# rare-resilience-ai/Osteosarcoma_DiffusionModel

Measured on AMD Instinct MI355X. Metric: synthetic patients/sec (full T-step reverse sample), higher is better.
Workload: dtype f32; 1 GPU; reverse sampling of conditional patients, T=1000, D=2000 (50 mut + 1900 expr + 50 pathway), hidden [256,512,256], 3 scenario conditions (BASELINE config 3); patients_per_gpu=100000, T=1000, parallelism=patients sharded over 1 GPU(s), no collective, sampler=chain, chunk_rows=65536, streams=2, graph=True

## Files before the change

osteosarcoma_diffusionmodel_amd/csrc/chain.h:

```cpp
#pragma once
#include "gemm_glds.h"
#include "epilogues.h"
#include "xpose.h"
#include "launch.h"

namespace osd {

constexpr int CHAIN_MAX_LAYERS = 24;
enum : int { CK_INPUT = 0, CK_GN32 = 1, CK_GN64 = 2, CK_POST = 3 };
enum : unsigned { CHAIN_OK = 0, CHAIN_TIMEOUT = 1, CHAIN_ABORT = 2 };

struct ChainLayer {
  const float* A; int lda;
  int K, K0;
  int F;
  int in0, ld0, in1, ld1;
  int out, ldo;
  int kind;
  const float* bias; const float* gamma; const float* beta;
};

struct ChainArgs {
  ChainLayer L[CHAIN_MAX_LAYERS];
  int n_layers;
  float* ws; long long ws_stride;
  float* x; int D;
  int n, n_tiles;
  int t_first, n_steps;
  unsigned base_done;
  const float* cproj; int ldc;
  const float* temb; int ldt;
  const float* coef;
  const float* z; int ldzz; long long z_step_stride; int z_t_first;
  uint64_t seed; uint32_t row_offset;
  float* mut_mask; int mutation_dim;
  unsigned* progress;
  unsigned* status;
  unsigned* queue;
  unsigned* cu_arrivals;
  int stagger;
  unsigned long long spin_budget;
  unsigned long long* stamps;
};

typedef __attribute__((address_space(1))) unsigned gu32;

__device__ __forceinline__ unsigned ld_relaxed_agent(const unsigned* p) {
  return __hip_atomic_load(p, __ATOMIC_RELAXED, __HIP_MEMORY_SCOPE_AGENT);
}
__device__ __forceinline__ void st_relaxed_agent(unsigned* p, unsigned v) {
  __hip_atomic_store(p, v, __ATOMIC_RELAXED, __HIP_MEMORY_SCOPE_AGENT);
}

__device__ __forceinline__ bool chain_wait(const unsigned* word, unsigned want, unsigned* status, unsigned long long budget, int lane) {
  if ((unsigned)__builtin_amdgcn_readfirstlane((int)ld_relaxed_agent(word)) >= want) return true;
  const unsigned long long t0 = __builtin_amdgcn_s_memrealtime();
  for (;;) {
    __builtin_amdgcn_s_sleep(32);
    if ((unsigned)__builtin_amdgcn_readfirstlane((int)ld_relaxed_agent(word)) >= want) return true;
    if ((unsigned)__builtin_amdgcn_readfirstlane((int)ld_relaxed_agent(status)) != CHAIN_OK) return false;
    if (__builtin_amdgcn_s_memrealtime() - t0 > budget) {
      if (lane == 0) st_relaxed_agent(status, CHAIN_TIMEOUT);
      return false;
    }
  }
}

constexpr int CHAIN_PRM_FLOATS = 512;

template <int NPB>
struct XposeRowsOut {
  const WaveXpose<NPB>& xp; float* out; int ldo;
  __device__ __forceinline__ void put(int fb, int pb, int q, int l31, int h, float4 v) const { (void)fb; xp.put(pb, q, l31, h, v); }
  __device__ __forceinline__ void flush(int fb, int lane) const { xp.template store_rows<false>(out + 32 * fb, ldo, lane, 0, 0); }
};
template <int NPB>
struct XposeRowsIn {
  const WaveXpose<NPB>& xp; const float* src; int ld;
  __device__ __forceinline__ void load(int fb, int lane) const { xp.template load_rows<false>(src + 32 * fb, ld, lane, 0, 0); }
  __device__ __forceinline__ float4 get(int fb, int pb, int q, int l31, int h) const { (void)fb; return xp.get(pb, q, l31, h); }
};

template <int GW, int NFB, int NPB, int PS, class Out>
__device__ __forceinline__ void chain_gn_silu(f32x16 (&acc)[NFB][NPB], const float* __restrict__ prm, int fl, const Out& o, int lane,
                                              unsigned long long* ts = nullptr) {
  static_assert(GW >= 8 && NFB * 32 >= GW, "wave must own whole groups");
  constexpr int RPG = GW / 2;
  constexpr int NG = NFB * 16 / RPG;
  const int l31 = lane & 31, h = lane >> 5;
#pragma unroll
  for (int fb = 0; fb < NFB; ++fb)
#pragma unroll
    for (int q = 0; q < 4; ++q) {
      const float4 bv = *reinterpret_cast<const float4*>(prm + fl + 32 * fb + 8 * q + 4 * h);
#pragma unroll
      for (int pb = 0; pb < NPB; ++pb) {
        acc[fb][pb][4 * q] += bv.x; acc[fb][pb][4 * q + 1] += bv.y;
        acc[fb][pb][4 * q + 2] += bv.z; acc[fb][pb][4 * q + 3] += bv.w;
      }
    }
  if (ts) { asm volatile("s_waitcnt vmcnt(0) lgkmcnt(0)" ::: "memory"); ts[0] = __builtin_amdgcn_s_memtime(); }
  float mean[NPB][NG], rstd[NPB][NG];
#pragma unroll
  for (int pb = 0; pb < NPB; ++pb)
#pragma unroll
    for (int g = 0; g < NG; ++g) {
      float s = 0.f;
#pragma unroll
      for (int j = 0; j < RPG; ++j) { const int Li = g * RPG + j; s += acc[Li / 16][pb][Li % 16]; }
      s += swap_halves(s);
      const float m = s * (1.0f / GW);
      float qs = 0.f;
#pragma unroll
      for (int j = 0; j < RPG; ++j) { const int Li = g * RPG + j; const float d = acc[Li / 16][pb][Li % 16] - m; qs = fmaf(d, d, qs); }
      qs += swap_halves(qs);
      mean[pb][g] = m;
      rstd[pb][g] = 1.0f / sqrtf(qs * (1.0f / GW) + GN_EPS);
    }
  if (ts) { asm volatile("s_nop 0" ::: "memory"); ts[1] = __builtin_amdgcn_s_memtime(); ts[2] = ts[1]; }
#pragma unroll
  for (int fb = 0; fb < NFB; ++fb) {
#pragma unroll
    for (int q = 0; q < 4; ++q) {
      const int f = fl + 32 * fb + 8 * q + 4 * h;
      const float4 gv = *reinterpret_cast<const float4*>(prm + PS + f);
      const float4 bev = *reinterpret_cast<const float4*>(prm + 2 * PS + f);
      const int g = (fb * 16 + 4 * q) / RPG;
#pragma unroll
      for (int pb = 0; pb < NPB; ++pb) {
        const float m = mean[pb][g], r = rstd[pb][g];
        float4 y;
        y.x = silu_f(fmaf((acc[fb][pb][4 * q] - m) * r, gv.x, bev.x));
        y.y = silu_f(fmaf((acc[fb][pb][4 * q + 1] - m) * r, gv.y, bev.y));
        y.z = silu_f(fmaf((acc[fb][pb][4 * q + 2] - m) * r, gv.z, bev.z));
        y.w = silu_f(fmaf((acc[fb][pb][4 * q + 3] - m) * r, gv.w, bev.w));
        o.put(fb, pb, q, l31, h, y);
      }
    }
    o.flush(fb, lane);
  }
}

template <int NFB, int NPB, int PS, class In, class Out>
__device__ __forceinline__ void chain_input(f32x16 (&acc)[NFB][NPB], const float* __restrict__ prm, int fl, const In& in, const Out& o, int lane) {
  const int l31 = lane & 31, h = lane >> 5;
#pragma unroll
  for (int fb = 0; fb < NFB; ++fb) {
    in.load(fb, lane);
#pragma unroll
    for (int q = 0; q < 4; ++q) {
      const int f = fl + 32 * fb + 8 * q + 4 * h;
      const float4 bv = *reinterpret_cast<const float4*>(prm + f);
      const float4 tv = *reinterpret_cast<const float4*>(prm + PS + f);
#pragma unroll
      for (int pb = 0; pb < NPB; ++pb) {
        const float4 cv = in.get(fb, pb, q, l31, h);
        float4 v;
        v.x = ((acc[fb][pb][4 * q] + bv.x) + tv.x) + cv.x;
        v.y = ((acc[fb][pb][4 * q + 1] + bv.y) + tv.y) + cv.y;
        v.z = ((acc[fb][pb][4 * q + 2] + bv.z) + tv.z) + cv.z;
        v.w = ((acc[fb][pb][4 * q + 3] + bv.w) + tv.w) + cv.w;
        o.put(fb, pb, q, l31, h, v);
      }
    }
    o.flush(fb, lane);
  }
}

#ifndef OSD_EXP
#define OSD_EXP 0
#endif
template <int NFB, int NPB, bool PRE = false, bool GUARD = true>
__device__ __forceinline__ void chain_posterior(f32x16 (&acc)[NFB][NPB], const float* __restrict__ prm, int fl, float* __restrict__ x, int ldx,
                                                int prow, int pcol, float cA, float cB, float cC, int t, const float* __restrict__ zrow, int ldzz,
                                                uint64_t seed, uint32_t row_id0, int f_glob, float* __restrict__ mut_mask, int mutation_dim,
                                                const WaveXpose<NPB>& xp, int lane, float4 (*pre)[4 * NPB] = nullptr) {
  const int l31 = lane & 31, h = lane >> 5;
  if (prow <= 0) return;
  const bool do_mask = t == 0 && mut_mask != nullptr;
#pragma unroll
  for (int fb = 0; fb < NFB; ++fb) {
    const int cols = pcol - 32 * fb;
    if (GUARD && cols <= 0) break;
    if constexpr (PRE) {
      if (!(OSD_EXP & 2)) {
        xp.commit_rows(*pre, lane);
        if (fb + 1 < NFB && cols - 32 > 0) xp.template issue_rows<GUARD>(*pre, x + 32 * (fb + 1), ldx, lane, prow, cols - 32);
      }
    } else {
      xp.template load_rows<GUARD>(x + 32 * fb, ldx, lane, prow, cols);
    }
#pragma unroll
    for (int pb = 0; pb < NPB; ++pb) {
      const int p = 32 * pb + l31;
      const int pc = (!GUARD || p < prow) ? p : prow - 1;
#pragma unroll
      for (int q = 0; q < 4; ++q) {
        const int fo = 32 * fb + 8 * q + 4 * h;
        const float4 bv = *reinterpret_cast<const float4*>(prm + fl + fo);
        const float e[4] = {acc[fb][pb][4 * q] + bv.x, acc[fb][pb][4 * q + 1] + bv.y, acc[fb][pb][4 * q + 2] + bv.z, acc[fb][pb][4 * q + 3] + bv.w};
        const float4 xq = xp.get(pb, q, l31, h);
        const float xv[4] = {xq.x, xq.y, xq.z, xq.w};
        float4 zz = make_float4(0.f, 0.f, 0.f, 0.f);
        if (t > 0 && cC != 0.f) {
          if (zrow) {
            const int fc = (!GUARD || fo < pcol - 4) ? fo : pcol - 4;
            zz = ldg4(zrow + (size_t)pc * ldzz + fc);
          } else if (!(OSD_EXP & 1)) {
            zz = randn4(seed, row_id0 + (uint32_t)p, (uint32_t)((f_glob + fo) >> 2), (uint32_t)t, TAG_POSTERIOR);
          }
        }
        const float zv[4] = {zz.x, zz.y, zz.z, zz.w};
        float o[4];
#pragma unroll
        for (int r = 0; r < 4; ++r) o[r] = fmaf(cA, xv[r], fmaf(cB, e[r], cC * zv[r]));
        if (do_mask && p < prow && fo < pcol && f_glob + fo < mutation_dim) {
          float* mrow = mut_mask + (size_t)p * mutation_dim;
#pragma unroll
          for (int r = 0; r < 4; ++r)
            if (f_glob + fo + r < mutation_dim) stg1(mrow + f_glob + fo + r, (o[r] > 0.5f) ? 1.0f : 0.0f);
        }
        xp.put(pb, q, l31, h, make_float4(o[0], o[1], o[2], o[3]));
      }
    }
    if (!(OSD_EXP & 4)) xp.template store_rows<GUARD>(x + 32 * fb, ldx, lane, prow, cols);
  }
}

#ifndef CHAIN_EPI_PRIO
#define CHAIN_EPI_PRIO 0
#endif
#ifndef CHAIN_BP
#define CHAIN_BP 128
#endif
#if CHAIN_BP == 128
typedef Tile<128, 128, 64, 64> ChainTile;
constexpr int CHAIN_WPS = 2;
#else
typedef Tile<128, 64, 64, 32> ChainTile;
constexpr int CHAIN_WPS = 3;
#endif
#ifdef OSD_DIAG
constexpr int CHAIN_KCNT = 12;
constexpr int CHAIN_STAMP_FLOATS = 2 * 4 * CHAIN_KCNT;
#else
constexpr int CHAIN_KCNT = 10;
constexpr int CHAIN_STAMP_FLOATS = 80;
#endif
constexpr int CHAIN_PRM_OFF = 2 * (ChainTile::BF * BK + ChainTile::BP * BK) + 4 + CHAIN_STAMP_FLOATS;
constexpr int CHAIN_LDS_BYTES = (CHAIN_PRM_OFF + 2 * CHAIN_PRM_FLOATS) * 4;
static_assert(CHAIN_PRM_OFF % 4 == 0, "parameter blocks are read as float4");

template <bool STAMP>
__global__ __launch_bounds__(NTHREADS, CHAIN_WPS) void chain_kernel(const ChainArgs* __restrict__ gp) {
  const ChainArgs& a = *gp;
  typedef ChainTile T;
  typedef GldsTile<T> G;
  static_assert(T::BF == 128 && T::BP % 32 == 0, "staging below assumes a 128-row weight image");
  constexpr int NW = NTHREADS / 64;
  constexpr int NPW = 16 / NW;
  constexpr int NPWB = T::BP / 8 / NW;
  constexpr int PROWS = 8 * NW;
  constexpr unsigned PBYTES = 1024u * NW;
  extern __shared__ __attribute__((aligned(16))) float smem[];
  float* As0 = smem;
  float* As1 = smem + G::A_ELEMS;
  float* Bs0 = smem + 2 * G::A_ELEMS;
  float* Bs1 = smem + 2 * G::A_ELEMS + G::B_ELEMS;
  volatile int& s_flag = *reinterpret_cast<volatile int*>(smem + 2 * (G::A_ELEMS + G::B_ELEMS));

  const int tid = threadIdx.x;
  const int lane = tid & 63;
  const int wave = __builtin_amdgcn_readfirstlane(tid >> 6);
  const int wf = (wave / T::NWP) * T::WF;
  const int wp = (wave % T::NWP) * T::WP;

  float* const ws = a.ws + (long long)blockIdx.x * a.ws_stride;
  WaveXpose<T::NPB> xp;
  {
    const int xo = wave * (T::NPB * 1024);
    xp.buf = xo < G::A_ELEMS ? As1 + xo : Bs1 + (xo - G::A_ELEMS);
  }
  float* const prm_base = smem + CHAIN_PRM_OFF;
  int pcur = 0;

  if (a.cu_arrivals && a.stagger > 0) {
    if (wave == 0) {
      const unsigned hw = __builtin_amdgcn_s_getreg(0xF804);
      const unsigned xcc = __builtin_amdgcn_s_getreg(0xF814) & 7;
      const unsigned key = (xcc << 8) | ((hw >> 8) & 0xFF);
      unsigned r = 0;
      if (lane == 0) r = atomicAdd(a.cu_arrivals + key, 1u);
      s_flag = __builtin_amdgcn_readfirstlane((int)(r & 1u));
    }
    __syncthreads();
    const int late = __builtin_amdgcn_readfirstlane(s_flag);
    __syncthreads();
    if (late) {
      const unsigned long long t0 = __builtin_amdgcn_s_memtime();
      while (__builtin_amdgcn_s_memtime() - t0 < (unsigned long long)a.stagger) __builtin_amdgcn_s_sleep(16);
    }
  }

  unsigned long long c_dep = 0, c_pro = 0, c_k = 0, c_epi = 0, c_units = 0;
  unsigned long long* const kcnt = reinterpret_cast<unsigned long long*>(smem + 2 * (G::A_ELEMS + G::B_ELEMS) + 4);
  if constexpr (STAMP) {
    if (tid < 4 * CHAIN_KCNT) kcnt[tid] = 0;
    __syncthreads();
  }
  const unsigned long long c_start = STAMP ? __builtin_amdgcn_s_memtime() : 0;
  const long long n_units = (long long)a.n_tiles * a.n_steps;
  int c_iter = 0;
  (void)c_iter;
  for (;;) {
    const unsigned long long td0 = STAMP ? __builtin_amdgcn_s_memtime() : 0;
#ifdef CHAIN_STATIC_UNITS
    static_assert(true, "");
    const long long u = (long long)blockIdx.x + (long long)c_iter * gridDim.x;
    ++c_iter;
#else
    if (wave == 0) {
      unsigned nu = 0;
      if (lane == 0) nu = atomicAdd(a.queue, 1u);
      s_flag = __builtin_amdgcn_readfirstlane((int)nu);
    }
    __syncthreads();
    const long long u = (unsigned)__builtin_amdgcn_readfirstlane(s_flag);
    __syncthreads();
#endif
    if (u >= n_units) break;
    const int tile = (int)(u % a.n_tiles);
    const int si = (int)(u / a.n_tiles);
    const int t = a.t_first - si;
    const int p0 = tile * T::BP;
    const int P = (a.n - p0 < T::BP) ? a.n - p0 : T::BP;

    if (wave == 0) {
      bool ok = (unsigned)__builtin_amdgcn_readfirstlane((int)ld_relaxed_agent(a.status)) == CHAIN_OK;
      if (ok && si > 0) {
        ok = chain_wait(a.progress + tile, a.base_done + (unsigned)si, a.status, a.spin_budget, lane);
        if (ok) __builtin_amdgcn_fence(__ATOMIC_ACQUIRE, "agent");
      }
      s_flag = ok ? 1 : 0;
      asm volatile("s_waitcnt vmcnt(0) lgkmcnt(0)" ::: "memory");
    }
    __syncthreads();
    const int go = __builtin_amdgcn_readfirstlane(s_flag);
    if (!go) return;
    if constexpr (STAMP) { c_dep += __builtin_amdgcn_s_memtime() - td0; ++c_units; }

    auto first_stage = [&](const ChainLayer& Lr, int f0n, bool do_a, bool do_b, int pb) {
      struct { const float* A; int lda, F, in0, ld0, K0, K; } Ln{Lr.A, Lr.lda, Lr.F, Lr.in0, Lr.ld0, Lr.K0, Lr.K};
      if (do_a && wave < 2) {
        const int kind = Lr.kind;
        const float* src = Lr.bias;
        if (wave == 1) src = Lr.beta;
        else if (lane >= 32) src = kind == CK_INPUT ? a.temb + (size_t)t * a.ldt : (kind == CK_POST ? Lr.bias : Lr.gamma);
        if (wave == 0 || (kind != CK_INPUT && kind != CK_POST)) {
          int f = f0n + 4 * (lane & 31);
          f = f < Ln.F - 4 ? f : Ln.F - 4;
          glds16(src + f, __builtin_amdgcn_readfirstlane(lds_addr(prm_base + pb * CHAIN_PRM_FLOATS) + (unsigned)wave * 1024u));
        }
      }
      const float* const xrows = a.x + (size_t)p0 * a.D;
      int ln = lane;
      asm volatile("" : "+v"(ln));
      const int r0 = wave * 8 + (ln >> 3);
      const int k4 = 4 * ((ln & 7) ^ ((r0 >> 1) & 7));
      const unsigned la = __builtin_amdgcn_readfirstlane(lds_addr(As0) + (unsigned)wave * 1024u);
      const unsigned lb = __builtin_amdgcn_readfirstlane(lds_addr(Bs0) + (unsigned)wave * 1024u);
      if (do_a) {
#pragma unroll
        for (int j = 0; j < NPW; ++j) {
          int rg = f0n + r0 + PROWS * j;
          rg = rg < Ln.F ? rg : Ln.F - 1;
          glds16(Ln.A + (size_t)rg * Ln.lda + k4, __builtin_amdgcn_readfirstlane(la + (unsigned)j * PBYTES));
        }
      }
      if (do_b) {
        const bool from_x = Ln.in0 < 0;
        const float* bb = from_x ? xrows : ws + Ln.in0;
        const int rows = from_x ? P : T::BP;
        const int kend = Ln.K0 < Ln.K ? Ln.K0 : Ln.K;
        const int k = k4 < kend - 4 ? k4 : kend - 4;
#pragma unroll
        for (int j = 0; j < NPWB; ++j) {
          int rg = r0 + PROWS * j;
          rg = rg < rows ? rg : rows - 1;
          glds16(bb + (size_t)rg * Ln.ld0 + k, __builtin_amdgcn_readfirstlane(lb + (unsigned)j * PBYTES));
        }
      }
    };
    unsigned long long tt0 = STAMP ? __builtin_amdgcn_s_memtime() : 0;
    first_stage(a.L[0], 0, true, true, pcur);
    asm volatile("s_waitcnt vmcnt(0)" ::: "memory");
    __syncthreads();

    for (int l = 0; l < a.n_layers; ++l) {
      const ChainLayer& L = a.L[l];
      const gfloat_ptr LA = uniform_ptr(L.A);
      const int Llda = L.lda, LK0 = L.K0, Lld0 = L.ld0, Lld1 = L.ld1;
      const int F = L.F, K = L.K;
      const float* const B0g = (L.in0 < 0) ? a.x + (size_t)p0 * a.D : ws + L.in0;
      const float* const B1g = ws + L.in1;
      const gfloat_ptr B0 = uniform_ptr(B0g), B1 = uniform_ptr(B1g);
      const int rowsB = (L.in0 < 0) ? P : T::BP;
      const int nk = (K + BK - 1) / BK;
      const int nft = (F + T::BF - 1) / T::BF;
      for (int ft = 0; ft < nft; ++ft) {
        const int f0 = ft * T::BF;
        int ln = lane;
        asm volatile("" : "+v"(ln));
        const int l31 = ln & 31, h = ln >> 5;
        int st_row[NPW], st_k4[NPW];
#pragma unroll
        for (int j = 0; j < NPW; ++j) {
          st_row[j] = (j * NW + wave) * 8 + (ln >> 3);
          st_k4[j] = 4 * ((ln & 7) ^ ((st_row[j] >> 1) & 7));
        }
        int a_rd[T::NFB], a_sw[T::NFB], b_rd[T::NPB], b_sw[T::NPB];
#pragma unroll
        for (int fb = 0; fb < T::NFB; ++fb) { const int R = wf + 32 * fb + l31; a_rd[fb] = R * BK; a_sw[fb] = h ^ ((R >> 1) & 7); }
#pragma unroll
        for (int pb = 0; pb < T::NPB; ++pb) { const int R = wp + 32 * pb + l31; b_rd[pb] = R * BK; b_sw[pb] = h ^ ((R >> 1) & 7); }
        unsigned offA[NPW], offB[NPWB];
#pragma unroll
        for (int j = 0; j < NPW; ++j) {
          int rg = f0 + st_row[j];
          rg = rg < F ? rg : F - 1;
          offA[j] = (unsigned)(rg * Llda + st_k4[j]) * 4u;
        }
#pragma unroll
        for (int j = 0; j < NPWB; ++j) {
          int rb = st_row[j];
          rb = rb < rowsB ? rb : rowsB - 1;
          offB[j] = (unsigned)(rb * Lld0 + st_k4[j]) * 4u;
        }
        int b_panel = 0;
        auto b_offsets_for = [&](int k0) {
          const int want = k0 < LK0 ? 0 : 1;
          if (want != b_panel) {
            b_panel = want;
            const int ld = want ? Lld1 : Lld0;
#pragma unroll
            for (int j = 0; j < NPWB; ++j) {
              int rb = st_row[j];
              rb = rb < rowsB ? rb : rowsB - 1;
              offB[j] = (unsigned)(rb * ld + st_k4[j]) * 4u;
            }
          }
        };
        struct StageCtx { gfloat_ptr sa, sb; unsigned la, lb; int k0; bool tail; };
        auto stage_begin = [&](int k0, float* As, float* Bs) {
          b_offsets_for(k0);
          const bool first = k0 < LK0;
          const int kend = first ? (LK0 < K ? LK0 : K) : K - LK0;
          const int kl = first ? k0 : k0 - LK0;
          StageCtx c;
          c.sa = LA + __builtin_amdgcn_readfirstlane(k0);
          c.sb = (first ? B0 : B1) + __builtin_amdgcn_readfirstlane(kl);
          c.la = __builtin_amdgcn_readfirstlane(lds_addr(As) + (unsigned)wave * 1024u);
          c.lb = __builtin_amdgcn_readfirstlane(lds_addr(Bs) + (unsigned)wave * 1024u);
          c.k0 = k0;
          c.tail = kl + BK > kend;
          return c;
        };
        auto piece = [&](const StageCtx& c, int j) {
          if (j < NPW) glds16s(c.sa, offA[j], __builtin_amdgcn_readfirstlane(c.la + (unsigned)j * PBYTES));
          else glds16s(c.sb, offB[j - NPW], __builtin_amdgcn_readfirstlane(c.lb + (unsigned)(j - NPW) * PBYTES));
        };
        auto stage_tail = [&](const StageCtx& c) {
#pragma unroll
          for (int j = 0; j < NPW; ++j) piece(c, j);
          const bool first = c.k0 < LK0;
          const int kend = first ? (LK0 < K ? LK0 : K) : K - LK0;
          const int kl = first ? c.k0 : c.k0 - LK0;
          const float* bb = first ? B0g : B1g;
          const int ld = first ? Lld0 : Lld1;
#pragma unroll
          for (int jb = 0; jb < NPWB; ++jb) {
            int k = kl + st_k4[jb];
            k = k < kend - 4 ? k : kend - 4;
            int rg = st_row[jb];
            rg = rg < rowsB ? rg : rowsB - 1;
            glds16(bb + (size_t)rg * ld + k, __builtin_amdgcn_readfirstlane(c.lb + (unsigned)jb * PBYTES));
          }
        };
        const unsigned long long tt1 = STAMP ? __builtin_amdgcn_s_memtime() : 0;

        unsigned long long c_kw = 0, c_kb = 0;
        (void)c_kw; (void)c_kb;
        f32x16 acc[T::NFB][T::NPB];
#pragma unroll
        for (int i = 0; i < T::NFB; ++i)
#pragma unroll
          for (int j = 0; j < T::NPB; ++j)
#pragma unroll
            for (int r = 0; r < 16; ++r) acc[i][j][r] = 0.f;

        float fa0[T::NFB][4], fb0[T::NPB][4], fa1[T::NFB][4], fb1[T::NPB][4];
        auto frags = [&](const float* Ac, const float* Bc, int i, float (&fa)[T::NFB][4], float (&fb)[T::NPB][4]) {
#pragma unroll
          for (int fb_ = 0; fb_ < T::NFB; ++fb_) {
            const float4 tq = *reinterpret_cast<const float4*>(&Ac[a_rd[fb_] + 4 * (a_sw[fb_] ^ (2 * i))]);
            fa[fb_][0] = tq.x; fa[fb_][1] = tq.y; fa[fb_][2] = tq.z; fa[fb_][3] = tq.w;
          }
#pragma unroll
          for (int pb = 0; pb < T::NPB; ++pb) {
            const float4 tq = *reinterpret_cast<const float4*>(&Bc[b_rd[pb] + 4 * (b_sw[pb] ^ (2 * i))]);
            fb[pb][0] = tq.x; fb[pb][1] = tq.y; fb[pb][2] = tq.z; fb[pb][3] = tq.w;
          }
        };
        auto quarter = [&](const float (&fa)[T::NFB][4], const float (&fb)[T::NPB][4]) {
#pragma unroll
          for (int e = 0; e < 4; ++e)
#pragma unroll
            for (int fb_ = 0; fb_ < T::NFB; ++fb_)
#pragma unroll
              for (int pb = 0; pb < T::NPB; ++pb)
                acc[fb_][pb] = __builtin_amdgcn_mfma_f32_32x32x2f32(fa[fb_][e], fb[pb][e], acc[fb_][pb], 0, 0, 0);
        };
        __builtin_amdgcn_sched_barrier(0);
        if (nk > 1) {
          const StageCtx c = stage_begin(BK, As1, Bs1);
          if (c.tail) stage_tail(c);
          else {
#pragma unroll
            for (int j = 0; j < NPW + NPWB; ++j) piece(c, j);
          }
        }
        frags(As0, Bs0, 0, fa0, fb0);
        __builtin_amdgcn_sched_barrier(0);
        for (int kt = 0; kt < nk; ++kt) {
          float* Ac = (kt & 1) ? As1 : As0;
          float* Bc = (kt & 1) ? Bs1 : Bs0;
          const float* An = (kt & 1) ? As0 : As1;
          const float* Bn = (kt & 1) ? Bs0 : Bs1;
          frags(Ac, Bc, 1, fa1, fb1);
          quarter(fa0, fb0);
          frags(Ac, Bc, 2, fa0, fb0);
          quarter(fa1, fb1);
          frags(Ac, Bc, 3, fa1, fb1);
          const bool ahead = kt + 2 < nk;
          StageCtx c{};
          if (ahead) c = stage_begin((kt + 2) * BK, Ac, Bc);
          const bool whole = ahead && !c.tail;
          quarter(fa0, fb0);
          __builtin_amdgcn_sched_barrier(0);
          const unsigned long long tw0 = STAMP ? __builtin_amdgcn_s_memtime() : 0;
          asm volatile("s_waitcnt vmcnt(0)" ::: "memory");
          const unsigned long long tw1 = STAMP ? __builtin_amdgcn_s_memtime() : 0;
          asm volatile("s_waitcnt lgkmcnt(0)" ::: "memory");
          __syncthreads();
          if constexpr (STAMP) { const unsigned long long tw2 = __builtin_amdgcn_s_memtime(); c_kw += tw1 - tw0; c_kb += tw2 - tw1; }
          __builtin_amdgcn_sched_barrier(0);
          if (ahead && c.tail) stage_tail(c);
          if (whole) {
#pragma unroll
            for (int j = 0; j < NPW + NPWB; ++j) piece(c, j);
          }
          if (kt + 1 < nk) frags(An, Bn, 0, fa0, fb0);
          __builtin_amdgcn_sched_barrier(0);
          quarter(fa1, fb1);
        }

        const unsigned long long tt2 = STAMP ? __builtin_amdgcn_s_memtime() : 0;
        const bool same_layer = ft + 1 < nft;
        const bool has_next = same_layer || l + 1 < a.n_layers;
        const int ln_next = same_layer ? l : l + 1;
        const int f0_next = same_layer ? f0 + T::BF : 0;
        const bool early_b = same_layer;
        if (has_next) first_stage(a.L[ln_next], f0_next, true, early_b, pcur ^ 1);
        const int fw = f0 + wf;
        const float* const prm = prm_base + pcur * CHAIN_PRM_FLOATS;
        pcur ^= 1;
        if (CHAIN_EPI_PRIO) __builtin_amdgcn_s_setprio(CHAIN_EPI_PRIO);
        const ChainArgs* ep = gp;
        asm volatile("" : "+s"(ep));
        const ChainArgs& e = *ep;
        unsigned long long ets[3] = {0, 0, 0};
        if (L.kind == CK_GN64) {
          const XposeRowsOut<T::NPB> o{xp, ws + L.out + (size_t)wp * L.ldo + fw, L.ldo};
          chain_gn_silu<64, T::NFB, T::NPB, 128>(acc, prm, wf, o, lane, STAMP ? ets : nullptr);
        } else if (L.kind == CK_GN32) {
          const XposeRowsOut<T::NPB> o{xp, ws + L.out + (size_t)wp * L.ldo + fw, L.ldo};
          chain_gn_silu<32, T::NFB, T::NPB, 128>(acc, prm, wf, o, lane, STAMP ? ets : nullptr);
        } else if (L.kind == CK_INPUT) {
          const XposeRowsIn<T::NPB> ci{xp, e.cproj + (size_t)(p0 + wp) * e.ldc + fw, e.ldc};
          const XposeRowsOut<T::NPB> o{xp, ws + L.out + (size_t)wp * L.ldo + fw, L.ldo};
          chain_input<T::NFB, T::NPB, 128>(acc, prm, wf, ci, o, lane);
        } else {
          const float* c = e.coef + 4 * t;
          const float cA = c[0], cB = c[1], cC = c[2];
          const float* zrow = e.z ? e.z + (long long)(e.z_t_first - t) * e.z_step_stride + (size_t)(p0 + wp) * e.ldzz + fw : nullptr;
          float* const mm = e.mut_mask ? e.mut_mask + (size_t)(p0 + wp) * e.mutation_dim : nullptr;
          chain_posterior<T::NFB, T::NPB>(acc, prm, wf, e.x + (size_t)(p0 + wp) * e.D + fw, e.D, P - wp, F - fw, cA, cB, cC, t, zrow, e.ldzz,
                                          e.seed, e.row_offset + (uint32_t)(p0 + wp), fw, mm, e.mutation_dim, xp, lane);
        }
        if (CHAIN_EPI_PRIO) __builtin_amdgcn_s_setprio(0);
        unsigned long long tt3 = 0, te1 = 0, te2 = 0, te3 = 0, te4 = 0;
        if constexpr (STAMP) te1 = __builtin_amdgcn_s_memtime();
        if (early_b) {
          if constexpr (STAMP) tt3 = __builtin_amdgcn_s_memtime();
          static_assert(4 * T::NFB * T::NPB == 16 || 4 * T::NFB * T::NPB == 8, "counted wait below is written for 16 or 8 stores");
          if (L.kind == CK_POST) asm volatile("s_waitcnt vmcnt(0)" ::: "memory");
          else if (4 * T::NFB * T::NPB == 16) asm volatile("s_waitcnt vmcnt(16)" ::: "memory");
          else asm volatile("s_waitcnt vmcnt(8)" ::: "memory");
          if constexpr (STAMP) te2 = __builtin_amdgcn_s_memtime();
          __syncthreads();
          if constexpr (STAMP) te3 = te4 = __builtin_amdgcn_s_memtime();
        } else {
          asm volatile("s_waitcnt vmcnt(0)" ::: "memory");
          if constexpr (STAMP) te2 = __builtin_amdgcn_s_memtime();
          __syncthreads();
          if constexpr (STAMP) tt3 = te3 = __builtin_amdgcn_s_memtime();
          if (has_next) {
            first_stage(a.L[ln_next], 0, false, true, 0);
            asm volatile("s_waitcnt vmcnt(0)" ::: "memory");
            __syncthreads();
          }
          if constexpr (STAMP) te4 = __builtin_amdgcn_s_memtime();
        }
        if constexpr (STAMP) {
          c_pro += tt1 - tt0; c_k += tt2 - tt1; c_epi += tt3 - tt2;
          tt0 = tt3;
          if (tid == 0) {
            unsigned long long* kc = kcnt + CHAIN_KCNT * L.kind;
            kc[0] += tt2 - tt1; kc[1] += te1 - tt2; kc[2] += te2 - te1; kc[3] += te3 - te2; kc[4] += te4 - te3; kc[5] += 1;
            if constexpr (CHAIN_KCNT >= 12) { kc[10] += c_kw; kc[11] += c_kb; }
            if (ets[0]) { kc[6] += ets[0] - tt2; kc[7] += ets[1] - ets[0]; kc[8] += ets[2] - ets[1]; kc[9] += te1 - ets[2]; }
          }
        }
      }
    }

    if (wave == 0) {
      __builtin_amdgcn_fence(__ATOMIC_RELEASE, "agent");
      asm volatile("s_waitcnt vmcnt(0)" ::: "memory");
      if (lane == 0) st_relaxed_agent(a.progress + tile, a.base_done + (unsigned)si + 1u);
    }
  }
  if (STAMP && a.stamps && tid == 0) {
    unsigned long long* o = a.stamps + (size_t)blockIdx.x * 64;
    o[0] = c_dep; o[1] = c_pro; o[2] = c_k; o[3] = c_epi; o[4] = __builtin_amdgcn_s_memtime() - c_start; o[5] = c_units;
    o[6] = __builtin_amdgcn_s_getreg(0xF804);
    o[7] = __builtin_amdgcn_s_getreg(0xF814) & 7;
    for (int i = 0; i < 4 * CHAIN_KCNT; ++i) o[8 + i] = kcnt[i];
  }
}

}
```

Baseline: 22820 patients/s.

## Use scalar-base addressing for chain loads/stores and peel zero-init into first MFMA

Rewrites the global-to-LDS staging, posterior x load/store and input-layer row transfers so a wave-uniform scalar base carries the row stride and each lane keeps only a small vector offset. This cuts per-lane 64-bit address arithmetic and VGPR pressure on the fast (unclamped) paths. The k-loop is unrolled by two with a compile-time odd/even buffer choice, and the explicit accumulator zeroing is replaced by feeding zero into the first MFMA. It also changes the swizzle to use st_row[0] for every j, which relies on all staged rows sharing the same swizzle.

```diff
diff --git a/osteosarcoma_diffusionmodel_amd/csrc/chain.h b/osteosarcoma_diffusionmodel_amd/csrc/chain.h
--- a/osteosarcoma_diffusionmodel_amd/csrc/chain.h
+++ b/osteosarcoma_diffusionmodel_amd/csrc/chain.h
@@ -44,6 +44,7 @@
 };
 
 typedef __attribute__((address_space(1))) unsigned gu32;
+template <bool B> struct BoolC { static constexpr bool value = B; };
 
 __device__ __forceinline__ unsigned ld_relaxed_agent(const unsigned* p) {
   return __hip_atomic_load(p, __ATOMIC_RELAXED, __HIP_MEMORY_SCOPE_AGENT);
@@ -81,6 +82,65 @@
   __device__ __forceinline__ float4 get(int fb, int pb, int q, int l31, int h) const { (void)fb; return xp.get(pb, q, l31, h); }
 };
 
+typedef __attribute__((address_space(1))) char gchar;
+__device__ __forceinline__ gfloat_ptr sbase_add(gfloat_ptr sbase, unsigned bytes) {
+  gfloat_ptr q = reinterpret_cast<gfloat_ptr>(reinterpret_cast<const gchar*>(sbase) + bytes);
+  asm("" : "+s"(q));
+  return q;
+}
+__device__ __forceinline__ v4f32 ldg4s(gfloat_ptr sbase, unsigned voff) {
+  return *reinterpret_cast<const gfloat4*>(reinterpret_cast<const gchar*>(sbase) + voff);
+}
+__device__ __forceinline__ void stg4s(gfloat_ptr sbase, unsigned voff, v4f32 v) {
+  *reinterpret_cast<gfloat4*>(const_cast<gchar*>(reinterpret_cast<const gchar*>(sbase)) + voff) = v;
+}
+template <int NPB, bool COLS>
+__device__ __forceinline__ void chain_store_rows(const WaveXpose<NPB>& xp, const float* g, int ld, int lane, int cols) {
+  const int c = lane & 7, r = lane >> 3, cr = c ^ r;
+  ld = __builtin_amdgcn_readfirstlane(ld);
+  const gfloat_ptr sb = uniform_ptr(g);
+  const unsigned step = (unsigned)ld * 32u;
+  const unsigned voff = (unsigned)(r * ld + 4 * c) * 4u;
+  const bool ok = !COLS || 4 * c < cols;
+#pragma unroll
+  for (int i0 = 0; i0 < 4 * NPB; i0 += 4) {
+    v4f32 v[4];
+#pragma unroll
+    for (int j = 0; j < 4; ++j) v[j] = *reinterpret_cast<const v4f32*>(xp.buf + r * 32 + (i0 + j) * 256 + 4 * (cr ^ ((i0 + j) & 7)));
+    if (ok) {
+#pragma unroll
+      for (int j = 0; j < 4; ++j) stg4s(sbase_add(sb, (unsigned)(i0 + j) * step), voff, v[j]);
+    }
+  }
+}
+template <int NPB, bool COLS>
+__device__ __forceinline__ void chain_load_rows(const WaveXpose<NPB>& xp, const float* g, int ld, int lane, int cols) {
+  const int c = lane & 7, r = lane >> 3, cr = c ^ r;
+  ld = __builtin_amdgcn_readfirstlane(ld);
+  const gfloat_ptr sb = uniform_ptr(g);
+  const unsigned step = (unsigned)ld * 32u;
+  int cc = 4 * c;
+  if (COLS) cc = cc < cols - 4 ? cc : cols - 4;
+  const unsigned voff = (unsigned)(r * ld + cc) * 4u;
+  v4f32 v[4 * NPB];
+#pragma unroll
+  for (int i = 0; i < 4 * NPB; ++i) v[i] = ldg4s(sbase_add(sb, (unsigned)i * step), voff);
+#pragma unroll
+  for (int i = 0; i < 4 * NPB; ++i) *reinterpret_cast<v4f32*>(xp.buf + r * 32 + i * 256 + 4 * (cr ^ (i & 7))) = v[i];
+}
+template <int NPB>
+struct ChainRowsOut {
+  const WaveXpose<NPB>& xp; float* out; int ldo;
+  __device__ __forceinline__ void put(int fb, int pb, int q, int l31, int h, float4 v) const { (void)fb; xp.put(pb, q, l31, h, v); }
+  __device__ __forceinline__ void flush(int fb, int lane) const { chain_store_rows<NPB, false>(xp, out + 32 * fb, ldo, lane, 0); }
+};
+template <int NPB>
+struct ChainRowsIn {
+  const WaveXpose<NPB>& xp; const float* src; int ld;
+  __device__ __forceinline__ void load(int fb, int lane) const { chain_load_rows<NPB, false>(xp, src + 32 * fb, ld, lane, 0); }
+  __device__ __forceinline__ float4 get(int fb, int pb, int q, int l31, int h) const { (void)fb; return xp.get(pb, q, l31, h); }
+};
+
 template <int GW, int NFB, int NPB, int PS, class Out>
 __device__ __forceinline__ void chain_gn_silu(f32x16 (&acc)[NFB][NPB], const float* __restrict__ prm, int fl, const Out& o, int lane,
                                               unsigned long long* ts = nullptr) {
@@ -170,7 +230,7 @@
 #ifndef OSD_EXP
 #define OSD_EXP 0
 #endif
-template <int NFB, int NPB, bool PRE = false, bool GUARD = true>
+template <int NFB, int NPB, bool PRE = false, bool GUARD = true, bool SADDR = false>
 __device__ __forceinline__ void chain_posterior(f32x16 (&acc)[NFB][NPB], const float* __restrict__ prm, int fl, float* __restrict__ x, int ldx,
                                                 int prow, int pcol, float cA, float cB, float cC, int t, const float* __restrict__ zrow, int ldzz,
                                                 uint64_t seed, uint32_t row_id0, int f_glob, float* __restrict__ mut_mask, int mutation_dim,
@@ -187,8 +247,12 @@
         xp.commit_rows(*pre, lane);
         if (fb + 1 < NFB && cols - 32 > 0) xp.template issue_rows<GUARD>(*pre, x + 32 * (fb + 1), ldx, lane, prow, cols - 32);
       }
+    } else if (SADDR && prow >= 32 * NPB && cols >= 4) {
+      chain_load_rows<NPB, true>(xp, x + 32 * fb, ldx, lane, cols);
     } else {
-      xp.template load_rows<GUARD>(x + 32 * fb, ldx, lane, prow, cols);
+      int ls = lane;
+      if (SADDR) asm volatile("" : "+v"(ls));
+      xp.template load_rows<GUARD>(x + 32 * fb, ldx, ls, prow, cols);
     }
 #pragma unroll
     for (int pb = 0; pb < NPB; ++pb) {
@@ -223,7 +287,14 @@
         xp.put(pb, q, l31, h, make_float4(o[0], o[1], o[2], o[3]));
       }
     }
-    if (!(OSD_EXP & 4)) xp.template store_rows<GUARD>(x + 32 * fb, ldx, lane, prow, cols);
+    if (!(OSD_EXP & 4)) {
+      if (SADDR && prow >= 32 * NPB && cols >= 4) chain_store_rows<NPB, true>(xp, x + 32 * fb, ldx, lane, cols);
+      else {
+        int ls = lane;
+        if (SADDR) asm volatile("" : "+v"(ls));
+        xp.template store_rows<GUARD>(x + 32 * fb, ldx, ls, prow, cols);
+      }
+    }
   }
 }
 
@@ -370,24 +441,41 @@
       const unsigned la = __builtin_amdgcn_readfirstlane(lds_addr(As0) + (unsigned)wave * 1024u);
       const unsigned lb = __builtin_amdgcn_readfirstlane(lds_addr(Bs0) + (unsigned)wave * 1024u);
       if (do_a) {
-#pragma unroll
-        for (int j = 0; j < NPW; ++j) {
-          int rg = f0n + r0 + PROWS * j;
-          rg = rg < Ln.F ? rg : Ln.F - 1;
-          glds16(Ln.A + (size_t)rg * Ln.lda + k4, __builtin_amdgcn_readfirstlane(la + (unsigned)j * PBYTES));
+        const gfloat_ptr sa = uniform_ptr(Ln.A);
+        if (f0n + T::BF <= Ln.F) {
+          const int lda = __builtin_amdgcn_readfirstlane(Ln.lda), f0s = __builtin_amdgcn_readfirstlane(f0n);
+          const unsigned o = (unsigned)(r0 * lda + k4) * 4u;
+#pragma unroll
+          for (int j = 0; j < NPW; ++j)
+            glds16s(sa + (unsigned)((f0s + PROWS * j) * lda), o, __builtin_amdgcn_readfirstlane(la + (unsigned)j * PBYTES));
+        } else {
+#pragma unroll
+          for (int j = 0; j < NPW; ++j) {
+            int rg = f0n + r0 + PROWS * j;
+            rg = rg < Ln.F ? rg : Ln.F - 1;
+            glds16s(sa, (unsigned)(rg * Ln.lda + k4) * 4u, __builtin_amdgcn_readfirstlane(la + (unsigned)j * PBYTES));
+          }
         }
       }
       if (do_b) {
         const bool from_x = Ln.in0 < 0;
-        const float* bb = from_x ? xrows : ws + Ln.in0;
+        const gfloat_ptr sb = uniform_ptr(from_x ? xrows : ws + Ln.in0);
         const int rows = from_x ? P : T::BP;
         const int kend = Ln.K0 < Ln.K ? Ln.K0 : Ln.K;
         const int k = k4 < kend - 4 ? k4 : kend - 4;
-#pragma unroll
-        for (int j = 0; j < NPWB; ++j) {
-          int rg = r0 + PROWS * j;
-          rg = rg < rows ? rg : rows - 1;
-          glds16(bb + (size_t)rg * Ln.ld0 + k, __builtin_amdgcn_readfirstlane(lb + (unsigned)j * PBYTES));
+        if (rows == T::BP) {
+          const int ld0 = __builtin_amdgcn_readfirstlane(Ln.ld0);
+          const unsigned o = (unsigned)(r0 * ld0 + k) * 4u;
+#pragma unroll
+          for (int j = 0; j < NPWB; ++j)
+            glds16s(sb + (unsigned)(PROWS * j * ld0), o, __builtin_amdgcn_readfirstlane(lb + (unsigned)j * PBYTES));
+        } else {
+#pragma unroll
+          for (int j = 0; j < NPWB; ++j) {
+            int rg = r0 + PROWS * j;
+            rg = rg < rows ? rg : rows - 1;
+            glds16s(sb, (unsigned)(rg * Ln.ld0 + k) * 4u, __builtin_amdgcn_readfirstlane(lb + (unsigned)j * PBYTES));
+          }
         }
       }
     };
@@ -416,7 +504,7 @@
 #pragma unroll
         for (int j = 0; j < NPW; ++j) {
           st_row[j] = (j * NW + wave) * 8 + (ln >> 3);
-          st_k4[j] = 4 * ((ln & 7) ^ ((st_row[j] >> 1) & 7));
+          st_k4[j] = 4 * ((ln & 7) ^ ((st_row[0] >> 1) & 7));
         }
         int a_rd[T::NFB], a_sw[T::NFB], b_rd[T::NPB], b_sw[T::NPB];
 #pragma unroll
@@ -424,23 +512,35 @@
 #pragma unroll
         for (int pb = 0; pb < T::NPB; ++pb) { const int R = wp + 32 * pb + l31; b_rd[pb] = R * BK; b_sw[pb] = h ^ ((R >> 1) & 7); }
         unsigned offA[NPW], offB[NPWB];
-#pragma unroll
-        for (int j = 0; j < NPW; ++j) {
-          int rg = f0 + st_row[j];
-          rg = rg < F ? rg : F - 1;
-          offA[j] = (unsigned)(rg * Llda + st_k4[j]) * 4u;
-        }
-#pragma unroll
-        for (int j = 0; j < NPWB; ++j) {
-          int rb = st_row[j];
-          rb = rb < rowsB ? rb : rowsB - 1;
-          offB[j] = (unsigned)(rb * Lld0 + st_k4[j]) * 4u;
+        if (f0 + T::BF <= F) {
+          const unsigned o = (unsigned)(st_row[0] * Llda + st_k4[0]) * 4u;
+#pragma unroll
+          for (int j = 0; j < NPW; ++j) offA[j] = o + (unsigned)((f0 + PROWS * j) * Llda) * 4u;
+        } else {
+#pragma unroll
+          for (int j = 0; j < NPW; ++j) {
+            int rg = f0 + st_row[j];
+            rg = rg < F ? rg : F - 1;
+            offA[j] = (unsigned)(rg * Llda + st_k4[j]) * 4u;
+          }
+        }
+        if (rowsB == T::BP) {
+          const unsigned o = (unsigned)(st_row[0] * Lld0 + st_k4[0]) * 4u;
+#pragma unroll
+          for (int j = 0; j < NPWB; ++j) offB[j] = o + (unsigned)(PROWS * j * Lld0) * 4u;
+        } else {
+#pragma unroll
+          for (int j = 0; j < NPWB; ++j) {
+            int rb = st_row[j];
+            rb = rb < rowsB ? rb : rowsB - 1;
+            offB[j] = (unsigned)(rb * Lld0 + st_k4[j]) * 4u;
+          }
         }
         int b_panel = 0;
         auto b_offsets_for = [&](int k0) {
           const int want = k0 < LK0 ? 0 : 1;
           if (want != b_panel) {
-            b_panel = want;
+            b_panel = __builtin_amdgcn_readfirstlane(want);
             const int ld = want ? Lld1 : Lld0;
 #pragma unroll
             for (int j = 0; j < NPWB; ++j) {
@@ -491,12 +591,6 @@
         unsigned long long c_kw = 0, c_kb = 0;
         (void)c_kw; (void)c_kb;
         f32x16 acc[T::NFB][T::NPB];
-#pragma unroll
-        for (int i = 0; i < T::NFB; ++i)
-#pragma unroll
-          for (int j = 0; j < T::NPB; ++j)
-#pragma unroll
-            for (int r = 0; r < 16; ++r) acc[i][j][r] = 0.f;
 
         float fa0[T::NFB][4], fb0[T::NPB][4], fa1[T::NFB][4], fb1[T::NPB][4];
         auto frags = [&](const float* Ac, const float* Bc, int i, float (&fa)[T::NFB][4], float (&fb)[T::NPB][4]) {
@@ -511,14 +605,15 @@
             fb[pb][0] = tq.x; fb[pb][1] = tq.y; fb[pb][2] = tq.z; fb[pb][3] = tq.w;
           }
         };
-        auto quarter = [&](const float (&fa)[T::NFB][4], const float (&fb)[T::NPB][4]) {
+        auto quarter = [&](const float (&fa)[T::NFB][4], const float (&fb)[T::NPB][4], auto first) {
+          const f32x16 zero = {};
 #pragma unroll
           for (int e = 0; e < 4; ++e)
 #pragma unroll
             for (int fb_ = 0; fb_ < T::NFB; ++fb_)
 #pragma unroll
               for (int pb = 0; pb < T::NPB; ++pb)
-                acc[fb_][pb] = __builtin_amdgcn_mfma_f32_32x32x2f32(fa[fb_][e], fb[pb][e], acc[fb_][pb], 0, 0, 0);
+                acc[fb_][pb] = __builtin_amdgcn_mfma_f32_32x32x2f32(fa[fb_][e], fb[pb][e], (decltype(first)::value && e == 0) ? zero : acc[fb_][pb], 0, 0, 0);
         };
         __builtin_amdgcn_sched_barrier(0);
         if (nk > 1) {
@@ -531,21 +626,22 @@
         }
         frags(As0, Bs0, 0, fa0, fb0);
         __builtin_amdgcn_sched_barrier(0);
-        for (int kt = 0; kt < nk; ++kt) {
-          float* Ac = (kt & 1) ? As1 : As0;
-          float* Bc = (kt & 1) ? Bs1 : Bs0;
-          const float* An = (kt & 1) ? As0 : As1;
-          const float* Bn = (kt & 1) ? Bs0 : Bs1;
+        auto kstep = [&](int kt, auto first, auto odd) __attribute__((always_inline)) {
+          constexpr bool ODD = decltype(odd)::value;
+          float* Ac = ODD ? As1 : As0;
+          float* Bc = ODD ? Bs1 : Bs0;
+          const float* An = ODD ? As0 : As1;
+          const float* Bn = ODD ? Bs0 : Bs1;
           frags(Ac, Bc, 1, fa1, fb1);
-          quarter(fa0, fb0);
+          quarter(fa0, fb0, first);
           frags(Ac, Bc, 2, fa0, fb0);
-          quarter(fa1, fb1);
+          quarter(fa1, fb1, BoolC<false>{});
           frags(Ac, Bc, 3, fa1, fb1);
           const bool ahead = kt + 2 < nk;
           StageCtx c{};
           if (ahead) c = stage_begin((kt + 2) * BK, Ac, Bc);
           const bool whole = ahead && !c.tail;
-          quarter(fa0, fb0);
+          quarter(fa0, fb0, BoolC<false>{});
           __builtin_amdgcn_sched_barrier(0);
           const unsigned long long tw0 = STAMP ? __builtin_amdgcn_s_memtime() : 0;
           asm volatile("s_waitcnt vmcnt(0)" ::: "memory");
@@ -561,7 +657,16 @@
           }
           if (kt + 1 < nk) frags(An, Bn, 0, fa0, fb0);
           __builtin_amdgcn_sched_barrier(0);
-          quarter(fa1, fb1);
+          quarter(fa1, fb1, BoolC<false>{});
+        };
+        kstep(0, BoolC<true>{}, BoolC<false>{});
+        {
+          int kt = 1;
+          for (; kt + 1 < nk; kt += 2) {
+            kstep(kt, BoolC<false>{}, BoolC<true>{});
+            kstep(kt + 1, BoolC<false>{}, BoolC<false>{});
+          }
+          if (kt < nk) kstep(kt, BoolC<false>{}, BoolC<true>{});
         }
 
         const unsigned long long tt2 = STAMP ? __builtin_amdgcn_s_memtime() : 0;
@@ -586,16 +691,16 @@
           const XposeRowsOut<T::NPB> o{xp, ws + L.out + (size_t)wp * L.ldo + fw, L.ldo};
           chain_gn_silu<32, T::NFB, T::NPB, 128>(acc, prm, wf, o, lane, STAMP ? ets : nullptr);
         } else if (L.kind == CK_INPUT) {
-          const XposeRowsIn<T::NPB> ci{xp, e.cproj + (size_t)(p0 + wp) * e.ldc + fw, e.ldc};
-          const XposeRowsOut<T::NPB> o{xp, ws + L.out + (size_t)wp * L.ldo + fw, L.ldo};
+          const ChainRowsIn<T::NPB> ci{xp, e.cproj + (size_t)(p0 + wp) * e.ldc + fw, e.ldc};
+          const ChainRowsOut<T::NPB> o{xp, ws + L.out + (size_t)wp * L.ldo + fw, L.ldo};
           chain_input<T::NFB, T::NPB, 128>(acc, prm, wf, ci, o, lane);
         } else {
           const float* c = e.coef + 4 * t;
           const float cA = c[0], cB = c[1], cC = c[2];
           const float* zrow = e.z ? e.z + (long long)(e.z_t_first - t) * e.z_step_stride + (size_t)(p0 + wp) * e.ldzz + fw : nullptr;
           float* const mm = e.mut_mask ? e.mut_mask + (size_t)(p0 + wp) * e.mutation_dim : nullptr;
-          chain_posterior<T::NFB, T::NPB>(acc, prm, wf, e.x + (size_t)(p0 + wp) * e.D + fw, e.D, P - wp, F - fw, cA, cB, cC, t, zrow, e.ldzz,
-                                          e.seed, e.row_offset + (uint32_t)(p0 + wp), fw, mm, e.mutation_dim, xp, lane);
+          chain_posterior<T::NFB, T::NPB, false, true, true>(acc, prm, wf, e.x + (size_t)(p0 + wp) * e.D + fw, e.D, P - wp, F - fw, cA, cB, cC, t,
+                                                             zrow, e.ldzz, e.seed, e.row_offset + (uint32_t)(p0 + wp), fw, mm, e.mutation_dim, xp, lane);
         }
         if (CHAIN_EPI_PRIO) __builtin_amdgcn_s_setprio(0);
         unsigned long long tt3 = 0, te1 = 0, te2 = 0, te3 = 0, te4 = 0;
```

Result: no change. 22950 patients/s, median of 6 (+0.6%).
